# jizongFox/MI-based-Regularized-Semi-supervised-Segmentation

Hardware: NVIDIA B200
Metric: iic_mi_loss_fwd_bwd_mpixels_per_s (higher is better)
Workload: dtype f32

## Files before the change

mi-based-regularized-semi-supervised-segmentation_b200/csrc/common.cuh:

```cuda
#pragma once
#include <cuda_runtime.h>
#include <stdint.h>
#include <stdio.h>
#include <string.h>

#include "../../include/iic_b200.h"

namespace iic {

void set_error(const char* fmt, ...);
const char* get_error();

#define IIC_CHECK_CUDA(expr)                                                               \
  do {                                                                                     \
    cudaError_t _e = (expr);                                                               \
    if (_e != cudaSuccess) {                                                               \
      ::iic::set_error("%s:%d: %s failed: %s", __FILE__, __LINE__, #expr,                  \
                       cudaGetErrorString(_e));                                            \
      return 1;                                                                            \
    }                                                                                      \
  } while (0)

#define IIC_REQUIRE(cond, ...)                                                             \
  do {                                                                                     \
    if (!(cond)) {                                                                         \
      ::iic::set_error(__VA_ARGS__);                                                       \
      return 2;                                                                            \
    }                                                                                      \
  } while (0)

#define IIC_CHECK_RC(expr)                                                                 \
  do {                                                                                     \
    const int _rc = (expr);                                                                \
    if (_rc != 0) return _rc;                                                              \
  } while (0)

int sm_count_cached(int device);
int current_device();

struct Options {
  int no_tma = 0;
  int no_tc = 0;
  int no_tc10 = 0;
  int no_fast = 0;
  int tcp_p1 = 0;
  int tcrb_p1 = 0;
  int tc10_force = 0;
  int no_tcj10 = 0;
  int tc10_tf32 = 0;
  int no_fused_epilogue = 0;
  int fin_last_cta_epilogue = 0;
  int xchg_timeout_ms = 0;
};
const Options& options();

inline size_t local_coeff_base_floats(int K, int pad, int n_patches) {
  const int T = 2 * pad + 1, Kp = (K + 3) & ~3;
  return (size_t)n_patches * K * T * T * Kp;
}
inline size_t local_coeff_image_offset(int K, int pad, int n_patches) {
  return (local_coeff_base_floats(K, pad, n_patches) + 255) & ~(size_t)255;
}

enum SlotLayoutKind { SLOT_STD = 0, SLOT_TC128 = 1, SLOT_PACKED = 2 };
struct SlotInfo {
  int layout;
  int n_slots;
  long long slot_stride;
  int nb;
};
__host__ __device__ inline size_t packed_slot_index(int mt, int m, int c, int nb) {
  return ((((size_t)mt * (nb / 8) + c / 8) * 2 + (c % 8) / 4) * 128 + m) * 4 + (c % 4);
}
__host__ __device__ inline long long tc128_out_index(long long e) {
  const long long w = e & 3, i = (e >> 2) & 127, jv = (e >> 9) & 7, ch = (e >> 12) & 3, d = e >> 14;
  return (d * 128 + i) * 128 + ch * 32 + jv * 4 + w;
}

int ensure_dyn_smem(const void* func, int bytes);

struct PatchGrid {
  int H, W;
  int ph, pw;
  int sh, sw;
  int nh, nw;
// ... 80 lines not shown
```

mi-based-regularized-semi-supervised-segmentation_b200/csrc/epilogue.cu:

```cuda
#include "epilogue.cuh"
#include "local_kernels.cuh"

namespace iic {

struct EpiWorkspace {
  unsigned int ticket;
  unsigned int pad_;
};

__global__ void __launch_bounds__(256) local_epilogue_kernel(
    const double* __restrict__ J, int K, int T, int n_patches, double lamda, float* __restrict__ loss_out,
    double* __restrict__ loss64_out, float* __restrict__ Wx, float* __restrict__ Wy,
    double* __restrict__ GA_out, int* __restrict__ flags, EpiWorkspace* ws) {
  extern __shared__ __align__(16) double sm[];
  double* partial_loss = reinterpret_cast<double*>(ws + 1);
  const int T2 = T * T;
  const int patch = blockIdx.x / T2, d = blockIdx.x % T2;
  const size_t KK = (size_t)K * K;
  const int Kp = (K + 3) & ~3;
  const int tid = threadIdx.x;
  const double scale = 1.0 / ((double)T2 * (double)n_patches);
  const double loss_d = local_epilogue_block(J + (size_t)patch * T2 * KK, K, T, d, lamda, scale,
                                             Wx + (size_t)patch * K * T2 * Kp, Wy + (size_t)patch * K * T2 * Kp,
                                             GA_out ? GA_out + ((size_t)patch * T2 + d) * KK : nullptr, sm);
// ... 80 lines not shown
}

struct GlobalStats { double S; };

__global__ void __launch_bounds__(1024) global_epilogue_kernel(const double* __restrict__ J, int K,
                                                               double lamb, int symmetric,
                                                               float* __restrict__ losses_out,
                                                               float* __restrict__ P_out,
                                                               int* __restrict__ flags) {
  extern __shared__ __align__(16) double sm[];
  global_epilogue_block(J, K, lamb, symmetric, losses_out, P_out, flags, sm);
}

constexpr int GLOBAL_BWD_STAGE_FLOATS = 2048;

__global__ void __launch_bounds__(256) global_backward_kernel(
    const float* __restrict__ x, long long x_sn, const float* __restrict__ y, long long y_sn, long long N,
    int K, const double* __restrict__ J, double lamb, int symmetric, const float* __restrict__ g_loss,
    const float* __restrict__ g_no_lamb, const float* __restrict__ gP, float* __restrict__ gx,
    float* __restrict__ gy, long long gx_sn, long long gy_sn,
    long long rows_per_cta) {
  extern __shared__ __align__(16) double sm[];
  double* scratch = sm;
  double* pi = sm + 40;
  double* pj = pi + K;
  double* gi = pj + K;
  double* gj = gi + K;
  double* Js = gj + K;
  float* GJ = reinterpret_cast<float*>(Js + (size_t)K * K);
  float* rows_s = GJ + (size_t)K * K;
  const int tid = threadIdx.x, nt = blockDim.x;
  const size_t KK = (size_t)K * K;
  const double eps = 1e-10;
  const long long r0 = (long long)blockIdx.x * rows_per_cta;
  long long r1 = r0 + rows_per_cta;
  if (r1 > N) r1 = N;
  const long long slab = (r1 - r0) * K;
  const bool staged_rows = slab <= GLOBAL_BWD_STAGE_FLOATS;
  if (staged_rows)
    for (long long e = tid; e < slab; e += nt) {
      const long long n = r0 + e / K;
      const int c = (int)(e % K);
      rows_s[e] = x[n * x_sn + c];
      rows_s[slab + e] = y[n * y_sn + c];
    }
  const double g1 = g_loss ? (double)g_loss[0] : 0.0, g2 = g_no_lamb ? (double)g_no_lamb[0] : 0.0;
  double part = 0.0;
  for (size_t e = tid; e < KK; e += nt) {
    const int i = (int)(e / K), j = (int)(e % K);
    const double v = symmetric ? (J[(size_t)i * K + j] + J[(size_t)j * K + i]) / 2.0 : J[(size_t)i * K + j];
    Js[e] = v;
    part += v;
  }
  const double S = block_sum(part, scratch);
  for (int k = tid; k < K; k += nt) {
    double r = 0.0, c = 0.0;
    for (int q = 0; q < K; ++q) {
      r += Js[(size_t)k * K + q];
      c += Js[(size_t)q * K + k];
    }
    pi[k] = r / S;
    pj[k] = c / S;
    gi[k] = log(pi[k] + eps) + pi[k] / (pi[k] + eps);
    gj[k] = log(pj[k] + eps) + pj[k] / (pj[k] + eps);
  }
  __syncthreads();
  double t_part = 0.0;
  for (size_t e = tid; e < KK; e += nt) {
    const int i = (int)(e / K), j = (int)(e % K);
    const double p = Js[e] / S;
    const double base = -log(p + eps) - p / (p + eps);
    const double mterm = gj[j] + gi[i];
    double v = g1 * (base + lamb * mterm) + g2 * (base + mterm);
    if (gP) v += (double)gP[e];
    Js[e] = v;
    t_part += v * p;
  }
  const double tot = block_sum(t_part, scratch);
  for (size_t e = tid; e < KK; e += nt) {
    const int i = (int)(e / K), j = (int)(e % K);
    double v;
    if (symmetric) v = ((Js[e] - tot) / S + (Js[(size_t)j * K + i] - tot) / S) / 2.0;
    else v = (Js[e] - tot) / S;
    GJ[e] = (float)v;
  }
  __syncthreads();
  const long long total = (r1 - r0) * K;
  for (long long e = tid; e < total; e += nt) {
    const long long n = r0 + e / K;
    const int c = (int)(e % K);
    const float* xr = staged_rows ? rows_s + (n - r0) * K : x + n * x_sn;
    const float* yr = staged_rows ? rows_s + slab + (n - r0) * K : y + n * y_sn;
    float ax = 0.f, ay = 0.f;
    for (int q = 0; q < K; ++q) {
      ax = fmaf(GJ[(size_t)c * K + q], yr[q], ax);
      ay = fmaf(GJ[(size_t)q * K + c], xr[q], ay);
    }
    gx[n * gx_sn + c] = ax;
    gy[n * gy_sn + c] = ay;
  }
}

static int global_grid(int device, long long N, long long* rows_per_cta) {
  int sms = sm_count_cached(device);
  if (sms <= 0) sms = 148;
  long long ctas = (N + 255) / 256;
  if (ctas > sms) ctas = sms;
  if (ctas < 1) ctas = 1;
  *rows_per_cta = (N + ctas - 1) / ctas;
// ... 67 lines not shown
    global_reduce_kernel<<<(K * K + 255) / 256, 256, 0, st>>>((const double*)workspace, ctas, K * K, J_out);
    IIC_CHECK_CUDA(cudaGetLastError());
  }
  return 0;
}

extern "C" int iic_global_epilogue(const double* J, int K, double lamb, int symmetric,
                                   float* losses_out, float* P_out, int* flags, void* stream) {
  cudaStream_t st = (cudaStream_t)stream;
  IIC_REQUIRE(J && K > 0, "iic_global_epilogue: bad arguments");
  IIC_REQUIRE(!losses_out || flags, "iic_global_epilogue: flags required with losses_out");
  const size_t smem = (40 + 2 * (size_t)K) * sizeof(double);
  int nt = K * K;
  nt = nt > 1024 ? 1024 : ((nt + 31) & ~31);
  global_epilogue_kernel<<<1, nt, smem, st>>>(J, K, lamb, symmetric, losses_out, P_out, flags);
  IIC_CHECK_CUDA(cudaGetLastError());
  return 0;
}

extern "C" int iic_global_backward(const float* x, long long x_sn, const float* y, long long y_sn,
                                   long long N, int K, const double* J, double lamb, int symmetric,
                                   const float* g_loss, const float* g_no_lamb, const float* gP, float* gx,
                                   float* gy, long long gx_sn, long long gy_sn, void* stream) {
  cudaStream_t st = (cudaStream_t)stream;
  IIC_REQUIRE(x && y && J && gx && gy, "iic_global_backward: null pointer");
  IIC_REQUIRE(N > 0 && K > 0 && K <= 128, "iic_global_backward: bad sizes N=%lld K=%d", N, K);
  long long rpc;
  const int ctas = global_grid(current_device(), N, &rpc);
  const size_t smem = (40 + 4 * (size_t)K + (size_t)K * K) * sizeof(double) + ((size_t)K * K + 2 * GLOBAL_BWD_STAGE_FLOATS) * sizeof(float);
  auto kern = global_backward_kernel;
  if (smem > 48 * 1024) IIC_CHECK_RC(ensure_dyn_smem((const void*)kern, (int)((40 + 4 * 128 + 128 * 128) * sizeof(double) + (128 * 128 + 2 * GLOBAL_BWD_STAGE_FLOATS) * sizeof(float))));
  if (gx_sn <= 0) gx_sn = K;
  if (gy_sn <= 0) gy_sn = K;
  kern<<<ctas, 256, smem, st>>>(x, x_sn, y, y_sn, N, K, J, lamb, symmetric, g_loss, g_no_lamb, gP, gx, gy, gx_sn, gy_sn, rpc);
  IIC_CHECK_CUDA(cudaGetLastError());
  return 0;
}
```

mi-based-regularized-semi-supervised-segmentation_b200/csrc/finish.cu:

```cuda
#include "epilogue.cuh"
#include "xchg.cuh"

namespace iic {

constexpr int FIN_MAX_ITEMS = 32;
constexpr int FIN_THREADS = 1024;
constexpr int FIN_WARPS = FIN_THREADS / 32;
constexpr int FIN_MAX_K = 32;
constexpr int FIN_MAX_UNITS = 1024;
constexpr int FIN_MAX_PATCHES = 256;
constexpr int FIN_SMALL_UNITS = 32;
constexpr int FIN_BIG_MAX_UNITS = 16384;
constexpr size_t FIN_WS_TICKETS = 64;
constexpr size_t FIN_WS_LOSSES = 256;

struct FinItem {
  const float* slots;
  const float* x;
  const float* y;
  long long x_sn, y_sn, N;
  double* J;
  float* loss_out;
  float* Wx;
  float* Wy;
// ... 205 lines not shown
    const int i = e / K, j = e - i * K;
    const double p = Jsym(i, j) * inv_S;
    if (it.P_out) it.P_out[e] = (float)p;
    const double lp = log(p + eps), lj = pj[j], li = pi[i];
    l1 += -p * (lp - lamb * lj - lamb * li);
    l2 += -p * (lp - lj - li);
  }
  const double L1 = warp_sum(l1), L2 = warp_sum(l2);
  if (lane == 0 && it.loss_out) {
    it.loss_out[0] = (float)L1;
    it.loss_out[1] = (float)L2;
    if ((L1 != L1 || L2 != L2) && flags) atomicOr(flags, IIC_FLAG_NAN_LOSS);
  }
  __syncwarp();
}

#ifdef IIC_FIN_TRACE
__device__ unsigned long long g_fin_trace[16];
__device__ __forceinline__ unsigned long long fin_now() { unsigned long long t; asm volatile("mov.u64 %0, %%globaltimer;" : "=l"(t)); return t; }
#define FIN_T(i) do { if (threadIdx.x == 0) g_fin_trace[i] = fin_now(); } while (0)
#else
#define FIN_T(i) do { } while (0)
#endif

__global__ void __launch_bounds__(FIN_THREADS, 1) finish_kernel(const __grid_constant__ FinBatch B) {
  __shared__ double sm[FIN_WARPS][33];
  __shared__ double unit_loss[FIN_MAX_UNITS];
  __shared__ double patch_min[FIN_MAX_PATCHES];
  __shared__ double wscratch[FIN_WARPS][3 * FIN_MAX_K];
  __shared__ double red_scratch[40];
  __shared__ unsigned long long seq_s;
  __shared__ int last_s;
  const int tid = threadIdx.x, wid = tid >> 5, lane = tid & 31;
#ifdef IIC_FIN_TRACE
  if (tid == 0) atomicMin(&g_fin_trace[0], fin_now());
#endif

  XchgHeader* hdr = nullptr;
  int par = 0;
  unsigned long long seq = 0;
  if (B.world > 1) {
    hdr = reinterpret_cast<XchgHeader*>(B.peers.base[B.rank]);
    if (tid == 0) seq_s = *reinterpret_cast<volatile unsigned long long*>(&hdr->seq) + 1;
    __syncthreads();
    seq = seq_s;
    par = (int)(seq & 1ull);
  }

  {
    long long base = 0;
    for (int i = 0; i < B.n; ++i) {
      const FinItem& it = B.it[i];
      const long long nu = item_units(it);
      long long first = blockIdx.x - (base % gridDim.x);
      if (first < 0) first += gridDim.x;
      for (long long u = first; u < nu; u += gridDim.x) {
        if (it.kind == IIC_ITEM_GLOBAL_ROWS) global_rows_unit(B, it, &sm[0][0], par);
        else reduce_unit(B, it, u, sm, par);
      }
      base += nu;
    }
  }
#ifdef IIC_FIN_TRACE
  if (tid == 0) atomicMax(&g_fin_trace[1], fin_now());
  if (tid == 0 && blockIdx.x == 0) g_fin_trace[7] = fin_now();
  if (tid == 0 && blockIdx.x == gridDim.x - 1) g_fin_trace[8] = fin_now();
#endif
  if (B.world > 1 && B.xchg_mode == 2) __threadfence_system(); else __threadfence();
  __syncthreads();
  if (tid == 0) last_s = (atomicAdd(B.ticket, 1u) == gridDim.x - 1) ? 1 : 0;
  __syncthreads();
  if (!last_s) return;
  __threadfence();
  FIN_T(2);

  if (B.world > 1) {
    if (B.xchg_mode == 2) {
      __threadfence_system();
    } else {
      for (long long e = tid; e < B.E_total; e += FIN_THREADS) {
        const double v = __ldcg(B.J_all + e);
        for (int p = 0; p < B.world; ++p) xchg_slot(B.peers.base[p], par, B.world, B.rank, B.capacity)[e] = v;
      }
      __syncthreads();
      if (tid < B.world) __threadfence_system();
    }
    if (tid < B.world) {
      XchgHeader* ph = reinterpret_cast<XchgHeader*>(B.peers.base[tid]);
      st_release_sys(&ph->flags[par][B.rank], seq);
    }
    if (B.xchg_mode == 2) {
      if (tid == 0) *B.ticket = 0;
      return;
    }
    if (tid < B.world) {
// ... 84 lines not shown
      double part = 0.0;
      for (int u = lane; u < nu; u += 32) part += unit_loss[ubase + u];
      double total = warp_sum(part);
      total *= 1.0 / ((double)nu);
      FIN_T(9);
      if (lane == 0) {
        it.loss_out[0] = (float)total;
        if (total != total && B.flags) atomicOr(B.flags, IIC_FLAG_NAN_LOSS);
      }
    }
  }
  FIN_T(6);
}

#ifdef IIC_FIN_TRACE
extern "C" int iic_debug_fin_trace(unsigned long long* host16, int reset) {
  if (reset) {
    unsigned long long z[16];
    for (int i = 0; i < 16; ++i) z[i] = 0;
    z[0] = ~0ull;
    return cudaMemcpyToSymbol(g_fin_trace, z, sizeof(z)) == cudaSuccess ? 0 : 1;
  }
  return cudaMemcpyFromSymbol(host16, g_fin_trace, 16 * sizeof(unsigned long long)) == cudaSuccess ? 0 : 1;
}
#endif

__global__ void __launch_bounds__(FIN_THREADS) xchg_sum_kernel(double* __restrict__ J_all, long long E_total, XchgPeers peers,
                                                               int rank, int world, long long capacity,
                                                               unsigned long long timeout_ns, int* __restrict__ flags,
                                                               unsigned int* __restrict__ ticket) {
  XchgHeader* hdr = reinterpret_cast<XchgHeader*>(peers.base[rank]);
  __shared__ unsigned long long seq_s;
  __shared__ int last_s;
  if (threadIdx.x == 0) seq_s = *reinterpret_cast<volatile unsigned long long*>(&hdr->seq) + 1;
  __syncthreads();
  const unsigned long long seq = seq_s;
  const int par = (int)(seq & 1ull);
  if (threadIdx.x < world && !xchg_wait_flag(hdr, par, threadIdx.x, seq, timeout_ns) && flags) atomicOr(flags, IIC_FLAG_XCHG_TIMEOUT);
  __syncthreads();
  const double* src = xchg_slot(peers.base[rank], par, world, 0, capacity);
  for (long long e = (long long)blockIdx.x * FIN_THREADS + threadIdx.x; e < E_total; e += (long long)gridDim.x * FIN_THREADS) {
    double s = 0.0;
    for (int r = 0; r < world; ++r) s += __ldcg(src + (size_t)r * capacity + e);
    J_all[e] = s;
  }
  __threadfence();
  __syncthreads();
  if (threadIdx.x == 0) last_s = (atomicAdd(ticket, 1u) == gridDim.x - 1) ? 1 : 0;
  __syncthreads();
  if (last_s && threadIdx.x == 0) {
    *ticket = 0;
    *reinterpret_cast<volatile unsigned long long*>(&hdr->seq) = seq;
  }
}

__global__ void __launch_bounds__(256) batched_epilogue_kernel(const __grid_constant__ FinBatch B, unsigned int* __restrict__ tickets,
                                                               double* __restrict__ unit_loss) {
  extern __shared__ __align__(16) double esm[];
  __shared__ int last_s;
  int item = 0, ubase = 0;
  for (; item < B.n; ++item) {
    const int nu = B.it[item].kind == IIC_ITEM_GLOBAL_ROWS ? 1 : B.it[item].n_patches * B.it[item].T * B.it[item].T;
    if ((int)blockIdx.x < ubase + nu) break;
    ubase += nu;
  }
  if (item >= B.n) return;
  const FinItem& it = B.it[item];
  if (it.kind == IIC_ITEM_GLOBAL_ROWS) {
    global_epilogue_block(it.J, it.K, it.lamda, it.symmetric, it.loss_out, it.P_out, B.flags, esm);
    return;
  }
  const int T2 = it.T * it.T, Kp = (it.K + 3) & ~3;
  const int u = (int)blockIdx.x - ubase, p = u / T2, d = u - p * T2, nu = it.n_patches * T2;
  const long long Eper = it.E / it.n_patches;
  const double scale = 1.0 / ((double)T2 * (double)it.n_patches);
  const double loss_d = local_epilogue_block(it.J + (size_t)p * Eper, it.K, it.T, d, it.lamda, scale,
                                             it.Wx + (size_t)p * it.K * T2 * Kp, it.Wy + (size_t)p * it.K * T2 * Kp, nullptr, esm);
  if (threadIdx.x == 0) {
    unit_loss[blockIdx.x] = loss_d;
    __threadfence();
    last_s = (atomicAdd(&tickets[item], 1u) == (unsigned)nu - 1) ? 1 : 0;
  }
  __syncthreads();
  if (last_s && threadIdx.x == 0) {
    __threadfence();
    const volatile double* pl = unit_loss + ubase;
    double total = 0.0;
    for (int q = 0; q < nu; ++q) total += pl[q];
    total *= scale;
    it.loss_out[0] = (float)total;
    if (total != total && B.flags) atomicOr(B.flags, IIC_FLAG_NAN_LOSS);
    tickets[item] = 0;
// ... 53 lines not shown
      d.nb = s.nb;
      d.T = 2 * s.pad + 1;
      d.n_patches = s.n_patches;
      d.E = (long long)s.n_patches * d.T * d.T * s.K * s.K;
      d.Wx = s.Wx;
      d.Wy = s.Wy;
      epi_units += (long long)s.n_patches * d.T * d.T;
      epi_patches += s.n_patches;
    } else {
      IIC_REQUIRE(s.x && s.y && s.N > 0, "iic_finish: global term %d is malformed", i);
      IIC_REQUIRE(s.K <= FIN_MAX_K * 4 && s.N <= (1 << 20), "iic_finish: global term %d too large for the direct joint", i);
      d.x = s.x; d.y = s.y; d.x_sn = s.x_sn; d.y_sn = s.y_sn; d.N = s.N;
      d.T = 1;
      d.n_patches = 1;
      d.E = (long long)s.K * s.K;
      d.symmetric = s.symmetric;
      d.check_simplex = s.check_simplex;
      d.P_out = s.P_out;
      epi_units += 1;
    }
    units += (d.kind == IIC_ITEM_GLOBAL_ROWS) ? 1 : (long long)d.n_patches * ((d.E / d.n_patches + 31) / 32);
    off += d.E;
  }
  IIC_REQUIRE(off == E_total, "iic_finish: the terms hold %lld joint entries, E_total says %lld", off, E_total);
  const bool small = fused && epi_units <= FIN_SMALL_UNITS && epi_patches <= FIN_MAX_PATCHES && E_total <= (long long)FIN_WARPS * 33;
  const bool last_cta_epilogue = small && options().fin_last_cta_epilogue;
  B.do_epilogue = last_cta_epilogue ? 1 : 0;
  B.xchg_mode = small ? 1 : 2;
  int sms = sm_count_cached(current_device());
  if (sms <= 0) sms = 148;
  long long grid = units < sms ? units : sms;
  if (grid < 1) grid = 1;
  unsigned int* tickets = reinterpret_cast<unsigned int*>(workspace);
  finish_kernel<<<(unsigned)grid, FIN_THREADS, 0, st>>>(B);
  IIC_CHECK_CUDA(cudaGetLastError());
  if (last_cta_epilogue) return 0;
  if (world > 1 && !small) {
    long long g2 = (E_total + FIN_THREADS - 1) / FIN_THREADS;
    if (g2 > sms) g2 = sms;
    xchg_sum_kernel<<<(unsigned)g2, FIN_THREADS, 0, st>>>(J_all, E_total, B.peers, rank, world, xchg_capacity, B.timeout_ns, flags,
                                                          tickets + 1);
    IIC_CHECK_CUDA(cudaGetLastError());
  }
  if (!want_epilogue) return 0;
  if (fused && epi_units <= FIN_BIG_MAX_UNITS) {
    int kmax = 1;
    for (int i = 0; i < n_items; ++i) kmax = items_host[i].K > kmax ? items_host[i].K : kmax;
    const size_t smem = (40 + 3 * (size_t)kmax) * sizeof(double);
    batched_epilogue_kernel<<<(unsigned)epi_units, 256, smem, st>>>(B, tickets + FIN_WS_TICKETS / sizeof(unsigned int),
                                                                    reinterpret_cast<double*>((unsigned char*)workspace + FIN_WS_LOSSES));
    IIC_CHECK_CUDA(cudaGetLastError());
    return 0;
  }
  for (int i = 0; i < n_items; ++i) {
    const iic_finish_item& s = items_host[i];
    const FinItem& d = B.it[i];
    if (s.kind == IIC_ITEM_LOCAL) {
      IIC_REQUIRE(s.epilogue_workspace, "iic_finish: term %d needs epilogue_workspace", i);
      IIC_CHECK_RC(iic_local_epilogue(d.J, s.K, s.pad, s.n_patches, s.lamda, s.loss_out, nullptr, s.Wx, s.Wy, nullptr, flags,
                                      s.epilogue_workspace, stream));
    } else {
      IIC_CHECK_RC(iic_global_epilogue(d.J, s.K, s.lamda, s.symmetric, s.loss_out, s.P_out, flags, stream));
    }
  }
  return 0;
}
```

mi-based-regularized-semi-supervised-segmentation_b200/csrc/local_bwd_tcrb10h.cu:

```cuda
#include <cuda_fp16.h>
#include <stdlib.h>

#include "common.cuh"
#include "local_kernels.cuh"
#include "tc_common.cuh"
#include "tma.cuh"

namespace iic {
namespace bwdrb10h {
using namespace tc;

constexpr int T = 3, PAD = 1;
constexpr int KP = 16;
constexpr int RMAX = 8;
constexpr int TBUF = 2 * RMAX * KP;
constexpr int APX = 272;
constexpr int MAXW = 248;
constexpr int A_CHUNK = APX * 16;
constexpr int A_SLOT = 4 * A_CHUNK;
constexpr int NA = 6;
constexpr int RAW_SLOT = 10 * 256 * 4;
constexpr int NRAW = 6;
constexpr int WROWS = T * KP;
constexpr int W_TILE = 2 * WROWS * 16;
// ... 82 lines not shown
__global__ void __launch_bounds__(FROM_LOGITS ? NTHREADS_FL : NTHREADS, 1)
local_bwd_tcrb10h_kernel(const __grid_constant__ CUtensorMap map0, const __grid_constant__ CUtensorMap map1, const Params P) {
  extern __shared__ __align__(1024) unsigned char smem_dyn[];
  __shared__ __align__(8) uint64_t raw_full[NRAW], raw_empty[NRAW], a_full[NA], a_empty[NA], w_full, accum_full[2], tmem_ready[2];
  __shared__ __align__(8) uint64_t l_full[NL], l_empty[NL];
  __shared__ uint32_t tmem_base_s;
  __shared__ float wmax_s[4];
  __shared__ float unscale_s;
  unsigned char* smem = smem_dyn + ((1024u - (smem_u32(smem_dyn) & 1023u)) & 1023u);
  unsigned char* a_ring = smem;
  unsigned char* w_img = smem + NA * A_SLOT;
  unsigned char* raw_ring = w_img + 2 * W_IMG;
  unsigned char* l_ring = raw_ring + NRAW * RAW_SLOT;
  const int wid = threadIdx.x >> 5, lane = threadIdx.x & 31;
  const long long rows_total = (long long)P.B * P.H;
  const long long R0 = (long long)blockIdx.x * rows_total / gridDim.x;
  const long long R1 = (long long)(blockIdx.x + 1) * rows_total / gridDim.x;
  const int share = (int)(R1 - R0);
  const int nch = (share + RMAX - 1) / RMAX;
  const int rc = nch > 0 ? (share + nch - 1) / nch : RMAX;
  const int SW = P.W + 8;
  const int raw_bytes = P.K * SW * 4;
  const int ntile = P.W > 128 ? 2 : 1;

  if (threadIdx.x == 0) {
    for (int s = 0; s < NRAW; ++s) { mbar_init(&raw_full[s], 1); mbar_init(&raw_empty[s], 4); }
    for (int s = 0; s < NA; ++s) { mbar_init(&a_full[s], 4); mbar_init(&a_empty[s], 2); }
    mbar_init(&w_full, 4);
    const int ndset_i = ntile == 2 ? 2 : 1;
    for (int s = 0; s < 2; ++s) { mbar_init(&accum_full[s], 4); mbar_init(&tmem_ready[s], 4 * ndset_i); }
    for (int s = 0; s < NL; ++s) { mbar_init(&l_full[s], 1); mbar_init(&l_empty[s], 4 * ndset_i); }
    mbar_fence_init();
  }
  if (wid == 3) {
    asm volatile("tcgen05.alloc.cta_group::1.sync.aligned.shared::cta.b32 [%0], %1;" ::"r"(smem_u32(&tmem_base_s)), "r"(512));
    asm volatile("tcgen05.relinquish_alloc_permit.cta_group::1.sync.aligned;");
  }
  asm volatile("tcgen05.fence::before_thread_sync;");
  __syncthreads();
  asm volatile("tcgen05.fence::after_thread_sync;");
  const uint32_t tmem_base = tmem_base_s;

  if (wid == 0) {
    if (lane == 0) {
      tma_prefetch_desc(&map0);
      tma_prefetch_desc(&map1);
      int t = 0, s = 0;
      unsigned sph = 0;
      for (int sweep = 0; sweep < 2; ++sweep)
      for (long long r = R0; r < R1;) {
        const Chunk c = next_chunk(r, R0, R1, P.H, rc);
        for (int q = c.q0; q < c.nr + T - 1; ++q, ++t) {
          { const int tt = t; (void)tt; TRACE(0, 0); }
          if (t >= NRAW) mbar_wait(&raw_empty[s], sph ^ 1u, 1);
          { const int tt = t; (void)tt; TRACE(0, 1); }
          mbar_arrive_expect_tx(&raw_full[s], raw_bytes);
          tma_load_4d(raw_ring + s * RAW_SLOT, sweep == 0 ? &map0 : &map1, &raw_full[s], -4, c.h0 - PAD + q, 0, c.n);
          if (++s == NRAW) { s = 0; sph ^= 1u; }
        }
        r += c.nr;
      }
    }
  } else if (wid == 3) {
    if (FROM_LOGITS && lane == 0) {
      int t = 0, s = 0;
      unsigned sph = 0;
      for (int sweep = 0; sweep < 2; ++sweep)
      for (long long r = R0; r < R1;) {
        const Chunk c = next_chunk(r, R0, R1, P.H, rc);
        for (int orow = 0; orow < c.nr; ++orow, ++t) {
          if (t >= NL) mbar_wait(&l_empty[s], sph ^ 1u, 9);
          mbar_arrive_expect_tx(&l_full[s], raw_bytes);
          tma_load_4d(l_ring + s * RAW_SLOT, sweep == 0 ? &map1 : &map0, &l_full[s], -4, c.h0 + orow, 0, c.n);
          if (++s == NL) { s = 0; sph ^= 1u; }
        }
        r += c.nr;
      }
    }
  } else if (wid == 1 || wid == 2 || wid == 12 || wid == 13) {
// ... 303 lines not shown
          for (int h = 0; h < nrow; ++h) {
            if (lane == 0) mbar_arrive(&l_empty[ls]);
            if (++ls == NL) { ls = 0; lph ^= 1u; }
          }
        }
      }
      r += c.nr;
      if (lane == 0 && wid == 14) CTRACE(4);
      zero_accumulators(buf);
      if (lane == 0 && wid == 14) CTRACE(5);
    }
  }
  asm volatile("tcgen05.fence::before_thread_sync;");
  __syncthreads();
  if (wid == 3) asm volatile("tcgen05.dealloc.cta_group::1.sync.aligned.b32 %0, %1;" ::"r"(tmem_base), "r"(512));
}

}

int local_bwd_tcrb10h_try(const LocalMaps& m, const float* Wx, const float* Wy, const LocalGrads& g, int from_logits,
                          float inv_temp, cudaStream_t st) {
  using namespace bwdrb10h;
  const int B = m.B, K = m.K, H = m.H, W = m.W, sms = m.sms;
  if ((K != 9 && K != 10) || m.pad != 1 || W % 4 != 0 || W > MAXW || W < 8) return -1;
  if ((long long)B * H < 8LL * sms && !options().tc10_force) return -1;
  CUtensorMap mx, my;
  if (!make_map_4d(&mx, m.x, m, W + 8, 1, K)) return -1;
  if (!make_map_4d(&my, m.y, m, W + 8, 1, K)) return -1;
  IIC_CHECK_RC(ensure_dyn_smem((const void*)(local_bwd_tcrb10h_kernel<false>), (int)(SMEM_BYTES)));
  IIC_CHECK_RC(ensure_dyn_smem((const void*)(local_bwd_tcrb10h_kernel<true>), (int)(SMEM_BYTES_FL)));
  const int Kp4 = (K + 3) & ~3;
  Params P{B, H, W, K, {Wx, Wy}, Kp4, g.grad_loss, {g.gx, g.gy}, {g.gx_sn, g.gy_sn}, from_logits, inv_temp, {m.x.p, m.y.p},
           {m.x.sn, m.y.sn}, {m.x.sc, m.y.sc}, {m.x.sh, m.y.sh}};
  if (from_logits) local_bwd_tcrb10h_kernel<true><<<sms, NTHREADS_FL, SMEM_BYTES_FL, st>>>(my, mx, P);
  else local_bwd_tcrb10h_kernel<false><<<sms, NTHREADS, SMEM_BYTES, st>>>(my, mx, P);
  IIC_CHECK_CUDA(cudaGetLastError());
  return 0;
}

}
```

mi-based-regularized-semi-supervised-segmentation_b200/csrc/local_fwd_tcj10.cu:

```cuda
#include <cuda_fp16.h>
#include <stdlib.h>

#include "common.cuh"
#include "local_kernels.cuh"
#include "tc_common.cuh"
#include "tma.cuh"

namespace iic {
namespace fwdtcj10 {
using namespace tc;

constexpr int PAD = 1;
constexpr int NPXB = 248;
constexpr int PAIRB = NPXB * 128;
constexpr int NXP = 4;
constexpr int NYP = 2;
constexpr int NSET = 2, NCOL = 192;
constexpr float SCALE = 1024.f;
constexpr int MAXW = 224;
constexpr int NTHREADS = 20 * 32;
constexpr int GROUP = 7 * 32;
constexpr int X_BYTES = (NXP + 1) * PAIRB;
constexpr int SMEM_BYTES = X_BYTES + NYP * PAIRB + 1024;

// ... 181 lines not shown
__global__ void __launch_bounds__(NTHREADS, 1) local_joint_tcj10_kernel(const Params P) {
  extern __shared__ __align__(1024) unsigned char smem_dyn[];
  __shared__ __align__(8) uint64_t x_full[NXP], x_free[NXP], y_full[NYP], y_done[NYP], set_free[NSET];
  __shared__ uint32_t tmem_base_s;
  unsigned char* smem = smem_dyn + ((1024u - (smem_u32(smem_dyn) & 1023u)) & 1023u);
  unsigned char* x_ring = smem;
  unsigned char* y_ring = smem + X_BYTES;
  const int wid = threadIdx.x >> 5, lane = threadIdx.x & 31;
  const long long rows_total = (long long)P.B * P.H;
  const long long R0 = (long long)blockIdx.x * rows_total / gridDim.x;
  const long long R1 = (long long)(blockIdx.x + 1) * rows_total / gridDim.x;
  const int ksteps = (P.W + 2 + 15) / 16;
  if (wid == 0) TCJ_T(0, 0);
#ifdef IIC_TCJ_DEBUG
  if (threadIdx.x == 0) { unsigned long long t; asm volatile("mov.u64 %0, %%globaltimer;" : "=l"(t)); g_tcj_cta[blockIdx.x][0] = t; }
#endif

  if (threadIdx.x == 0) {
    for (int s = 0; s < NXP; ++s) { mbar_init(&x_full[s], 7); mbar_init(&x_free[s], 2); }
    for (int s = 0; s < NYP; ++s) { mbar_init(&y_full[s], 7); mbar_init(&y_done[s], 1); }
    for (int s = 0; s < NSET; ++s) mbar_init(&set_free[s], 4);
    mbar_fence_init();
  }
  if (wid == 14) {
    asm volatile("tcgen05.alloc.cta_group::1.sync.aligned.shared::cta.b32 [%0], %1;" ::"r"(smem_u32(&tmem_base_s)), "r"(512));
    asm volatile("tcgen05.relinquish_alloc_permit.cta_group::1.sync.aligned;");
  }
  for (int e = threadIdx.x; e < (X_BYTES + NYP * PAIRB) / 16; e += NTHREADS) reinterpret_cast<uint4*>(smem)[e] = make_uint4(0, 0, 0, 0);
  asm volatile("fence.proxy.async.shared::cta;" ::: "memory");
  asm volatile("tcgen05.fence::before_thread_sync;");
  __syncthreads();
  asm volatile("tcgen05.fence::after_thread_sync;");
  const uint32_t tmem_base = tmem_base_s;
  if (wid == 0) TCJ_T(0, 1);

  if (wid < 14) {
    if (P.K == 10) {
      if (wid < 7) stage_pairs<false, true>(P, R0, R1, x_ring, x_ring + NXP * PAIRB, x_full, x_free);
      else stage_pairs<true, true>(P, R0, R1, y_ring, nullptr, y_full, y_done);
    } else {
      if (wid < 7) stage_pairs<false, false>(P, R0, R1, x_ring, x_ring + NXP * PAIRB, x_full, x_free);
      else stage_pairs<true, false>(P, R0, R1, y_ring, nullptr, y_full, y_done);
    }
  } else {
    const uint32_t idesc = (1u << 4) | (1u << 15) | (1u << 16) | ((uint32_t)(NCOL >> 3) << 17) | (8u << 24);
    const int a = wid & 3;
    const uint32_t lane_base = tmem_base + ((uint32_t)(a * 32) << 16);
    float tot[3][2][10];
#pragma unroll
    for (int s = 0; s < 3; ++s)
#pragma unroll
      for (int yr = 0; yr < 2; ++yr)
#pragma unroll
        for (int j = 0; j < 10; ++j) tot[s][yr][j] = 0.f;

    auto issue = [&](int yq, int ql, int xpbase, bool last_of_chunk) {
      const int ys = yq % NYP;
      const int xp1 = xpbase + ql + 1;
      TCJ_T(2, yq);
      mbar_wait(&y_full[ys], (unsigned)(yq / NYP) & 1u, 5);
      mbar_wait(&x_full[xp1 % NXP], (unsigned)(xp1 / NXP) & 1u, 6);
      if (yq >= NSET && !TCJ_DBG(128)) mbar_wait(&set_free[yq % NSET], (unsigned)((yq - NSET) / NSET) & 1u, 7);
      asm volatile("tcgen05.fence::after_thread_sync;");
      TCJ_T(1, yq);
      if (lane == 0) {
        const int xs = (xpbase + ql) % NXP;
// ... 24 lines not shown
#pragma unroll
        for (int yr = 0; yr < 2; ++yr) {
          const uint32_t col = lane_base + (uint32_t)(st * NCOL + s * 64 + yr * 32);
          asm volatile("tcgen05.ld.sync.aligned.32x32b.x16.b32 {%0, %1, %2, %3, %4, %5, %6, %7, %8, %9, %10, %11, %12, %13, %14, %15}, [%16];"
                       : "=r"(v[yr][0]), "=r"(v[yr][1]), "=r"(v[yr][2]), "=r"(v[yr][3]), "=r"(v[yr][4]), "=r"(v[yr][5]),
                         "=r"(v[yr][6]), "=r"(v[yr][7]), "=r"(v[yr][8]), "=r"(v[yr][9]), "=r"(v[yr][10]), "=r"(v[yr][11]),
                         "=r"(v[yr][12]), "=r"(v[yr][13]), "=r"(v[yr][14]), "=r"(v[yr][15])
                       : "r"(col));
          asm volatile("tcgen05.ld.sync.aligned.32x32b.x4.b32 {%0, %1, %2, %3}, [%4];"
                       : "=r"(v[yr][16]), "=r"(v[yr][17]), "=r"(v[yr][18]), "=r"(v[yr][19])
                       : "r"(col + 16));
        }
        asm volatile("tcgen05.wait::ld.sync.aligned;" ::: "memory");
#pragma unroll
        for (int yr = 0; yr < 2; ++yr)
#pragma unroll
          for (int j = 0; j < 10; ++j) tot[s][yr][j] += __uint_as_float(v[yr][j]) + __uint_as_float(v[yr][10 + j]);
      }
      asm volatile("tcgen05.fence::before_thread_sync;");
      __syncwarp();
      if (lane == 0) mbar_arrive(&set_free[st]);
    };

    int yq = 0, xpbase = 0;
    for (long long r = R0; r < R1;) {
      const Chunk c = chunk_at(r, R1, P.H);
      for (int ql = 0; ql < c.npy; ++ql, ++yq) {
        if (wid < 16) { if ((yq & 1) == (wid & 1)) issue(yq, ql, xpbase, ql == c.npy - 1); }
        else drain(yq);
      }
      xpbase += c.npy + 1;
      r += c.nr;
    }
    if (wid >= 16) {
    if (wid == 16) TCJ_T(0, 2);
    float* stage = reinterpret_cast<float*>(smem);
#pragma unroll
    for (int s = 0; s < 3; ++s)
#pragma unroll
      for (int yr = 0; yr < 2; ++yr) {
        const int dy = a - yr;
#pragma unroll
        for (int j = 0; j < 10; ++j) {
          const float full = tot[s][yr][j] + __shfl_down_sync(0xffffffffu, tot[s][yr][j], 10);
          if (lane < 10 && dy >= 0 && dy < 3) stage[((yr * 9 + dy * 3 + (2 - s)) * 10 + lane) * 10 + j] = full;
        }
      }
    asm volatile("bar.sync 1, 128;" ::: "memory");
    float* slot = P.partial + (size_t)blockIdx.x * (9 * P.K * P.K);
    const int tid = threadIdx.x - 16 * 32;
    for (int e = tid; e < 9 * P.K * P.K; e += 128) {
      const int d = e / (P.K * P.K), ij = e - d * P.K * P.K;
      const int i = ij / P.K, j = ij - i * P.K;
      const int o = (d * 10 + i) * 10 + j;
      slot[e] = (stage[o] + stage[900 + o]) * (1.f / (SCALE * SCALE));
    }
    if (wid == 16) TCJ_T(0, 3);
    }
  }
  asm volatile("tcgen05.fence::before_thread_sync;");
  __syncthreads();
#ifdef IIC_TCJ_DEBUG
  if (threadIdx.x == 0) { unsigned long long t; asm volatile("mov.u64 %0, %%globaltimer;" : "=l"(t)); g_tcj_cta[blockIdx.x][1] = t; }
#endif
  if (wid == 14) asm volatile("tcgen05.dealloc.cta_group::1.sync.aligned.b32 %0, %1;" ::"r"(tmem_base), "r"(512));
}

}

int local_joint_tcj10_try(const LocalMaps& m, float* partial, int max_ctas, SlotInfo* slots, int* flags, int* checked,
                          int from_logits, float inv_temp, cudaStream_t st) {
  using namespace fwdtcj10;
  const int B = m.B, K = m.K, H = m.H, W = m.W;
  *checked = 0;
  if (m.pad != PAD || K < 2 || K > 10 || W < 8 || W > MAXW) return -1;
  if (from_logits && K != 10) return -1;
  const long long rows = (long long)B * H;
  if (rows < 8LL * max_ctas) return -1;
  Params P;
  P.x = m.x.p; P.x_sn = m.x.sn; P.x_sc = m.x.sc; P.x_sh = m.x.sh;
  P.y = m.y.p; P.y_sn = m.y.sn; P.y_sc = m.y.sc; P.y_sh = m.y.sh;
  P.B = B; P.H = H; P.W = W; P.K = K;
  P.partial = partial;
  P.flags = from_logits ? nullptr : flags;
  P.from_logits = from_logits;
  P.inv_temp = inv_temp;
  auto rows16 = [&](const View4& v) {
    return (reinterpret_cast<uintptr_t>(v.p) & 15) == 0 && v.sn % 4 == 0 && v.sc % 4 == 0 && v.sh % 4 == 0;
  };
  if (W % 4 != 0 || !rows16(m.x) || !rows16(m.y)) return -1;
#ifdef IIC_TCJ_DEBUG
  P.dbg = 0;
#endif
  *checked = P.flags != nullptr;
  *slots = SlotInfo{SLOT_STD, max_ctas, (long long)9 * K * K, 0};
  IIC_CHECK_RC(ensure_dyn_smem((const void*)local_joint_tcj10_kernel, SMEM_BYTES));
  local_joint_tcj10_kernel<<<max_ctas, NTHREADS, SMEM_BYTES, st>>>(P);
  IIC_CHECK_CUDA(cudaGetLastError());
  return 0;
}

}
```

mi-based-regularized-semi-supervised-segmentation_b200/csrc/runtime.cu:

```cuda
#include <stdarg.h>
#include <stdlib.h>

#include <mutex>
#include <unordered_map>

#include "common.cuh"

namespace iic {

static thread_local char g_err[512] = "";
void set_error(const char* fmt, ...) {
  va_list ap;
  va_start(ap, fmt);
  vsnprintf(g_err, sizeof(g_err), fmt, ap);
  va_end(ap);
}
const char* get_error() { return g_err; }

int current_device() {
  int d = -1;
  if (cudaGetDevice(&d) != cudaSuccess) return -1;
  return d;
}
int sm_count_cached(int device) {
  static int cache[64];
  if (device < 0 || device >= 64) return -1;
  if (cache[device] > 0) return cache[device];
  int v = 0;
  if (cudaDeviceGetAttribute(&v, cudaDevAttrMultiProcessorCount, device) != cudaSuccess) {
    set_error("cudaDeviceGetAttribute(MultiProcessorCount, %d) failed: %s", device,
              cudaGetErrorString(cudaGetLastError()));
    return -1;
  }
  cache[device] = v;
  return v;
}

struct OptionEntry { const char* name; const char* env; int Options::*field; };
static const OptionEntry kOptions[] = {
    {"no_tma", "IIC_B200_NO_TMA", &Options::no_tma},
    {"no_tc", "IIC_B200_NO_TC", &Options::no_tc},
    {"no_tc10", "IIC_B200_NO_TC10", &Options::no_tc10},
    {"no_fast", "IIC_B200_NO_FAST", &Options::no_fast},
    {"tcp_p1", "IIC_B200_TCP_P1", &Options::tcp_p1},
    {"tcrb_p1", "IIC_B200_TCRB_P1", &Options::tcrb_p1},
    {"tc10_force", "IIC_B200_TC10_FORCE", &Options::tc10_force},
    {"no_tcj10", "IIC_B200_NO_TCJ10", &Options::no_tcj10},
    {"tc10_tf32", "IIC_B200_TC10_TF32", &Options::tc10_tf32},
    {"no_fused_epilogue", "IIC_B200_NO_FUSED_EPILOGUE", &Options::no_fused_epilogue},
    {"fin_last_cta_epilogue", "IIC_B200_FIN_LAST_CTA_EPILOGUE", &Options::fin_last_cta_epilogue},
    {"xchg_timeout_ms", "IIC_B200_XCHG_TIMEOUT_MS", &Options::xchg_timeout_ms},
};
static Options g_options;
static std::once_flag g_options_once;
static void load_options() {
  g_options.xchg_timeout_ms = 600000;
  for (const OptionEntry& e : kOptions) {
    const char* v = getenv(e.env);
    if (v && *v) {
      const int n = atoi(v);
      g_options.*(e.field) = (n != 0 || v[0] == '0') ? n : 1;
    }
  }
}
Options& options_mut() {
  std::call_once(g_options_once, load_options);
  return g_options;
}
const Options& options() { return options_mut(); }

int ensure_dyn_smem(const void* func, int bytes) {
  static std::mutex mu;
  static std::unordered_map<const void*, unsigned long long> done;
  const int dev = current_device();
  if (dev < 0 || dev >= 64) {
    set_error("ensure_dyn_smem: no current CUDA device");
    return 1;
  }
  std::lock_guard<std::mutex> lock(mu);
  unsigned long long& mask = done[func];
  if (mask & (1ull << dev)) return 0;
  IIC_CHECK_CUDA(cudaFuncSetAttribute(func, cudaFuncAttributeMaxDynamicSharedMemorySize, bytes));
  mask |= 1ull << dev;
  return 0;
// ... 28 lines not shown
```

Baseline: 10160.

## Launch pipeline kernels with programmatic dependent launch to overlap prologues

Adds a PDL launch helper that uses cudaLaunchKernelExC with programmatic stream serialization, and switches the forward joint, finish, exchange, epilogue and backward kernels to it. Each kernel calls griddepcontrol.wait after its setup (barrier init, TMEM alloc, descriptor prefetch) and signals dependents early, so a kernel's prologue can overlap the tail of the kernel before it. The global backward kernel also computes its loss-independent terms before waiting, uses __ldcg loads, and picks 128 threads for small K. The cost is added ordering subtlety: any read of upstream data placed before the wait would be a race.

Result: faster. 10510 (median of 6 runs) (+3.4%).

```diff
diff --git a/mi-based-regularized-semi-supervised-segmentation_b200/csrc/common.cuh b/mi-based-regularized-semi-supervised-segmentation_b200/csrc/common.cuh
--- a/mi-based-regularized-semi-supervised-segmentation_b200/csrc/common.cuh
+++ b/mi-based-regularized-semi-supervised-segmentation_b200/csrc/common.cuh
@@ -3,6 +3,10 @@
 #include <stdint.h>
 #include <stdio.h>
 #include <string.h>
+
+#include <tuple>
+#include <type_traits>
+#include <utility>
 
 #include "../../include/iic_b200.h"
 
@@ -38,6 +42,21 @@
 int sm_count_cached(int device);
 int current_device();
 
+int launch_pdl_args(const void* func, dim3 grid, dim3 block, size_t smem, cudaStream_t st, void** args);
+
+template <typename... P, typename... A>
+int launch_pdl(void (*kernel)(P...), dim3 grid, dim3 block, size_t smem, cudaStream_t st, A&&... args) {
+  static_assert(sizeof...(P) == sizeof...(A), "launch_pdl: argument count");
+  std::tuple<std::remove_cv_t<std::remove_reference_t<P>>...> v(std::forward<A>(args)...);
+  return std::apply([&](auto&... a) {
+    void* p[] = {static_cast<void*>(&a)...};
+    return launch_pdl_args(reinterpret_cast<const void*>(kernel), grid, block, smem, st, p);
+  }, v);
+}
+
+__device__ __forceinline__ void pdl_wait() { asm volatile("griddepcontrol.wait;" ::: "memory"); }
+__device__ __forceinline__ void pdl_launch_dependents() { asm volatile("griddepcontrol.launch_dependents;" ::: "memory"); }
+
 struct Options {
   int no_tma = 0;
   int no_tc = 0;
@@ -51,6 +70,7 @@
   int no_fused_epilogue = 0;
   int fin_last_cta_epilogue = 0;
   int xchg_timeout_ms = 0;
+  int no_pdl = 0;
 };
 const Options& options();
 
diff --git a/mi-based-regularized-semi-supervised-segmentation_b200/csrc/epilogue.cu b/mi-based-regularized-semi-supervised-segmentation_b200/csrc/epilogue.cu
--- a/mi-based-regularized-semi-supervised-segmentation_b200/csrc/epilogue.cu
+++ b/mi-based-regularized-semi-supervised-segmentation_b200/csrc/epilogue.cu
@@ -136,6 +136,11 @@
   const int tid = threadIdx.x, nt = blockDim.x;
   const size_t KK = (size_t)K * K;
   const double eps = 1e-10;
+  const bool early = KK <= (size_t)nt;
+  if (!early) {
+    pdl_wait();
+    pdl_launch_dependents();
+  }
   const long long r0 = (long long)blockIdx.x * rows_per_cta;
   long long r1 = r0 + rows_per_cta;
   if (r1 > N) r1 = N;
@@ -145,14 +150,13 @@
     for (long long e = tid; e < slab; e += nt) {
       const long long n = r0 + e / K;
       const int c = (int)(e % K);
-      rows_s[e] = x[n * x_sn + c];
-      rows_s[slab + e] = y[n * y_sn + c];
-    }
-  const double g1 = g_loss ? (double)g_loss[0] : 0.0, g2 = g_no_lamb ? (double)g_no_lamb[0] : 0.0;
+      rows_s[e] = __ldcg(x + n * x_sn + c);
+      rows_s[slab + e] = __ldcg(y + n * y_sn + c);
+    }
   double part = 0.0;
   for (size_t e = tid; e < KK; e += nt) {
     const int i = (int)(e / K), j = (int)(e % K);
-    const double v = symmetric ? (J[(size_t)i * K + j] + J[(size_t)j * K + i]) / 2.0 : J[(size_t)i * K + j];
+    const double v = symmetric ? (__ldcg(J + (size_t)i * K + j) + __ldcg(J + (size_t)j * K + i)) / 2.0 : __ldcg(J + (size_t)i * K + j);
     Js[e] = v;
     part += v;
   }
@@ -170,15 +174,38 @@
   }
   __syncthreads();
   double t_part = 0.0;
-  for (size_t e = tid; e < KK; e += nt) {
-    const int i = (int)(e / K), j = (int)(e % K);
-    const double p = Js[e] / S;
-    const double base = -log(p + eps) - p / (p + eps);
-    const double mterm = gj[j] + gi[i];
-    double v = g1 * (base + lamb * mterm) + g2 * (base + mterm);
-    if (gP) v += (double)gP[e];
-    Js[e] = v;
-    t_part += v * p;
+  if (early) {
+    const size_t e = tid;
+    double p = 0.0, gl = 0.0, g1p = 0.0;
+    if (e < KK) {
+      const int i = (int)(e / K), j = (int)(e % K);
+      p = Js[e] / S;
+      const double base = -log(p + eps) - p / (p + eps);
+      const double mterm = gj[j] + gi[i];
+      gl = base + lamb * mterm;
+      g1p = base + mterm;
+    }
+    pdl_wait();
+    pdl_launch_dependents();
+    const double g1 = g_loss ? (double)g_loss[0] : 0.0, g2 = g_no_lamb ? (double)g_no_lamb[0] : 0.0;
+    if (e < KK) {
+      double v = g1 * gl + g2 * g1p;
+      if (gP) v += (double)gP[e];
+      Js[e] = v;
+      t_part += v * p;
+    }
+  } else {
+    const double g1 = g_loss ? (double)g_loss[0] : 0.0, g2 = g_no_lamb ? (double)g_no_lamb[0] : 0.0;
+    for (size_t e = tid; e < KK; e += nt) {
+      const int i = (int)(e / K), j = (int)(e % K);
+      const double p = Js[e] / S;
+      const double base = -log(p + eps) - p / (p + eps);
+      const double mterm = gj[j] + gi[i];
+      double v = g1 * (base + lamb * mterm) + g2 * (base + mterm);
+      if (gP) v += (double)gP[e];
+      Js[e] = v;
+      t_part += v * p;
+    }
   }
   const double tot = block_sum(t_part, scratch);
   for (size_t e = tid; e < KK; e += nt) {
@@ -312,7 +339,7 @@
   if (smem > 48 * 1024) IIC_CHECK_RC(ensure_dyn_smem((const void*)kern, (int)((40 + 4 * 128 + 128 * 128) * sizeof(double) + (128 * 128 + 2 * GLOBAL_BWD_STAGE_FLOATS) * sizeof(float))));
   if (gx_sn <= 0) gx_sn = K;
   if (gy_sn <= 0) gy_sn = K;
-  kern<<<ctas, 256, smem, st>>>(x, x_sn, y, y_sn, N, K, J, lamb, symmetric, g_loss, g_no_lamb, gP, gx, gy, gx_sn, gy_sn, rpc);
-  IIC_CHECK_CUDA(cudaGetLastError());
-  return 0;
-}
+  const int nt = K * K <= 128 ? 128 : 256;
+  return launch_pdl(kern, ctas, nt, smem, st, x, x_sn, y, y_sn, N, K, J, lamb, symmetric, g_loss, g_no_lamb, gP, gx, gy, gx_sn,
+                    gy_sn, rpc);
+}
diff --git a/mi-based-regularized-semi-supervised-segmentation_b200/csrc/finish.cu b/mi-based-regularized-semi-supervised-segmentation_b200/csrc/finish.cu
--- a/mi-based-regularized-semi-supervised-segmentation_b200/csrc/finish.cu
+++ b/mi-based-regularized-semi-supervised-segmentation_b200/csrc/finish.cu
@@ -261,6 +261,7 @@
   __shared__ unsigned long long seq_s;
   __shared__ int last_s;
   const int tid = threadIdx.x, wid = tid >> 5, lane = tid & 31;
+  pdl_wait();
 #ifdef IIC_FIN_TRACE
   if (tid == 0) atomicMin(&g_fin_trace[0], fin_now());
 #endif
@@ -290,6 +291,7 @@
       base += nu;
     }
   }
+  if (B.world == 1 && !B.do_epilogue) pdl_launch_dependents();
 #ifdef IIC_FIN_TRACE
   if (tid == 0) atomicMax(&g_fin_trace[1], fin_now());
   if (tid == 0 && blockIdx.x == 0) g_fin_trace[7] = fin_now();
@@ -440,6 +442,7 @@
   XchgHeader* hdr = reinterpret_cast<XchgHeader*>(peers.base[rank]);
   __shared__ unsigned long long seq_s;
   __shared__ int last_s;
+  pdl_wait();
   if (threadIdx.x == 0) seq_s = *reinterpret_cast<volatile unsigned long long*>(&hdr->seq) + 1;
   __syncthreads();
   const unsigned long long seq = seq_s;
@@ -452,6 +455,7 @@
     for (int r = 0; r < world; ++r) s += __ldcg(src + (size_t)r * capacity + e);
     J_all[e] = s;
   }
+  pdl_launch_dependents();
   __threadfence();
   __syncthreads();
   if (threadIdx.x == 0) last_s = (atomicAdd(ticket, 1u) == gridDim.x - 1) ? 1 : 0;
@@ -466,6 +470,8 @@
                                                                double* __restrict__ unit_loss) {
   extern __shared__ __align__(16) double esm[];
   __shared__ int last_s;
+  pdl_wait();
+  pdl_launch_dependents();
   int item = 0, ubase = 0;
   for (; item < B.n; ++item) {
     const int nu = B.it[item].kind == IIC_ITEM_GLOBAL_ROWS ? 1 : B.it[item].n_patches * B.it[item].T * B.it[item].T;
@@ -585,25 +591,21 @@
   long long grid = units < sms ? units : sms;
   if (grid < 1) grid = 1;
   unsigned int* tickets = reinterpret_cast<unsigned int*>(workspace);
-  finish_kernel<<<(unsigned)grid, FIN_THREADS, 0, st>>>(B);
-  IIC_CHECK_CUDA(cudaGetLastError());
+  IIC_CHECK_RC(launch_pdl(finish_kernel, (unsigned)grid, FIN_THREADS, 0, st, B));
   if (last_cta_epilogue) return 0;
   if (world > 1 && !small) {
     long long g2 = (E_total + FIN_THREADS - 1) / FIN_THREADS;
     if (g2 > sms) g2 = sms;
-    xchg_sum_kernel<<<(unsigned)g2, FIN_THREADS, 0, st>>>(J_all, E_total, B.peers, rank, world, xchg_capacity, B.timeout_ns, flags,
-                                                          tickets + 1);
-    IIC_CHECK_CUDA(cudaGetLastError());
+    IIC_CHECK_RC(launch_pdl(xchg_sum_kernel, (unsigned)g2, FIN_THREADS, 0, st, J_all, E_total, B.peers, rank, world, xchg_capacity,
+                            B.timeout_ns, flags, tickets + 1));
   }
   if (!want_epilogue) return 0;
   if (fused && epi_units <= FIN_BIG_MAX_UNITS) {
     int kmax = 1;
     for (int i = 0; i < n_items; ++i) kmax = items_host[i].K > kmax ? items_host[i].K : kmax;
     const size_t smem = (40 + 3 * (size_t)kmax) * sizeof(double);
-    batched_epilogue_kernel<<<(unsigned)epi_units, 256, smem, st>>>(B, tickets + FIN_WS_TICKETS / sizeof(unsigned int),
-                                                                    reinterpret_cast<double*>((unsigned char*)workspace + FIN_WS_LOSSES));
-    IIC_CHECK_CUDA(cudaGetLastError());
-    return 0;
+    return launch_pdl(batched_epilogue_kernel, (unsigned)epi_units, 256, smem, st, B, tickets + FIN_WS_TICKETS / sizeof(unsigned int),
+                      reinterpret_cast<double*>((unsigned char*)workspace + FIN_WS_LOSSES));
   }
   for (int i = 0; i < n_items; ++i) {
     const iic_finish_item& s = items_host[i];
diff --git a/mi-based-regularized-semi-supervised-segmentation_b200/csrc/local_bwd_tcrb10h.cu b/mi-based-regularized-semi-supervised-segmentation_b200/csrc/local_bwd_tcrb10h.cu
--- a/mi-based-regularized-semi-supervised-segmentation_b200/csrc/local_bwd_tcrb10h.cu
+++ b/mi-based-regularized-semi-supervised-segmentation_b200/csrc/local_bwd_tcrb10h.cu
@@ -138,6 +138,10 @@
     for (int s = 0; s < NL; ++s) { mbar_init(&l_full[s], 1); mbar_init(&l_empty[s], 4 * ndset_i); }
     mbar_fence_init();
   }
+  if (wid == 0 && lane == 0) {
+    tma_prefetch_desc(&map0);
+    tma_prefetch_desc(&map1);
+  }
   if (wid == 3) {
     asm volatile("tcgen05.alloc.cta_group::1.sync.aligned.shared::cta.b32 [%0], %1;" ::"r"(smem_u32(&tmem_base_s)), "r"(512));
     asm volatile("tcgen05.relinquish_alloc_permit.cta_group::1.sync.aligned;");
@@ -146,11 +150,11 @@
   __syncthreads();
   asm volatile("tcgen05.fence::after_thread_sync;");
   const uint32_t tmem_base = tmem_base_s;
+  pdl_wait();
+  pdl_launch_dependents();
 
   if (wid == 0) {
     if (lane == 0) {
-      tma_prefetch_desc(&map0);
-      tma_prefetch_desc(&map1);
       int t = 0, s = 0;
       unsigned sph = 0;
       for (int sweep = 0; sweep < 2; ++sweep)
@@ -520,10 +524,8 @@
   const int Kp4 = (K + 3) & ~3;
   Params P{B, H, W, K, {Wx, Wy}, Kp4, g.grad_loss, {g.gx, g.gy}, {g.gx_sn, g.gy_sn}, from_logits, inv_temp, {m.x.p, m.y.p},
            {m.x.sn, m.y.sn}, {m.x.sc, m.y.sc}, {m.x.sh, m.y.sh}};
-  if (from_logits) local_bwd_tcrb10h_kernel<true><<<sms, NTHREADS_FL, SMEM_BYTES_FL, st>>>(my, mx, P);
-  else local_bwd_tcrb10h_kernel<false><<<sms, NTHREADS, SMEM_BYTES, st>>>(my, mx, P);
-  IIC_CHECK_CUDA(cudaGetLastError());
-  return 0;
-}
-
-}
+  if (from_logits) return launch_pdl(local_bwd_tcrb10h_kernel<true>, sms, NTHREADS_FL, SMEM_BYTES_FL, st, my, mx, P);
+  return launch_pdl(local_bwd_tcrb10h_kernel<false>, sms, NTHREADS, SMEM_BYTES, st, my, mx, P);
+}
+
+}
diff --git a/mi-based-regularized-semi-supervised-segmentation_b200/csrc/local_fwd_tcj10.cu b/mi-based-regularized-semi-supervised-segmentation_b200/csrc/local_fwd_tcj10.cu
--- a/mi-based-regularized-semi-supervised-segmentation_b200/csrc/local_fwd_tcj10.cu
+++ b/mi-based-regularized-semi-supervised-segmentation_b200/csrc/local_fwd_tcj10.cu
@@ -237,6 +237,7 @@
   __syncthreads();
   asm volatile("tcgen05.fence::after_thread_sync;");
   const uint32_t tmem_base = tmem_base_s;
+  pdl_wait();
   if (wid == 0) TCJ_T(0, 1);
 
   if (wid < 14) {
@@ -327,6 +328,7 @@
       xpbase += c.npy + 1;
       r += c.nr;
     }
+    if (wid < 16) pdl_launch_dependents();
     if (wid >= 16) {
     if (wid == 16) TCJ_T(0, 2);
     float* stage = reinterpret_cast<float*>(smem);
@@ -390,9 +392,7 @@
   *checked = P.flags != nullptr;
   *slots = SlotInfo{SLOT_STD, max_ctas, (long long)9 * K * K, 0};
   IIC_CHECK_RC(ensure_dyn_smem((const void*)local_joint_tcj10_kernel, SMEM_BYTES));
-  local_joint_tcj10_kernel<<<max_ctas, NTHREADS, SMEM_BYTES, st>>>(P);
-  IIC_CHECK_CUDA(cudaGetLastError());
-  return 0;
-}
-
-}
+  return launch_pdl(local_joint_tcj10_kernel, max_ctas, NTHREADS, SMEM_BYTES, st, P);
+}
+
+}
diff --git a/mi-based-regularized-semi-supervised-segmentation_b200/csrc/runtime.cu b/mi-based-regularized-semi-supervised-segmentation_b200/csrc/runtime.cu
--- a/mi-based-regularized-semi-supervised-segmentation_b200/csrc/runtime.cu
+++ b/mi-based-regularized-semi-supervised-segmentation_b200/csrc/runtime.cu
@@ -36,6 +36,21 @@
   return v;
 }
 
+int launch_pdl_args(const void* func, dim3 grid, dim3 block, size_t smem, cudaStream_t st, void** args) {
+  cudaLaunchAttribute attr;
+  attr.id = cudaLaunchAttributeProgrammaticStreamSerialization;
+  attr.val.programmaticStreamSerializationAllowed = 1;
+  cudaLaunchConfig_t cfg = {};
+  cfg.gridDim = grid;
+  cfg.blockDim = block;
+  cfg.dynamicSmemBytes = smem;
+  cfg.stream = st;
+  cfg.attrs = &attr;
+  cfg.numAttrs = options().no_pdl ? 0 : 1;
+  IIC_CHECK_CUDA(cudaLaunchKernelExC(&cfg, func, args));
+  return 0;
+}
+
 struct OptionEntry { const char* name; const char* env; int Options::*field; };
 static const OptionEntry kOptions[] = {
     {"no_tma", "IIC_B200_NO_TMA", &Options::no_tma},
@@ -50,6 +65,7 @@
     {"no_fused_epilogue", "IIC_B200_NO_FUSED_EPILOGUE", &Options::no_fused_epilogue},
     {"fin_last_cta_epilogue", "IIC_B200_FIN_LAST_CTA_EPILOGUE", &Options::fin_last_cta_epilogue},
     {"xchg_timeout_ms", "IIC_B200_XCHG_TIMEOUT_MS", &Options::xchg_timeout_ms},
+    {"no_pdl", "IIC_B200_NO_PDL", &Options::no_pdl},
 };
 static Options g_options;
 static std::once_flag g_options_once;
```
